# david-gimeno/tailored-avsr

Measured on AMD Instinct MI355X. Metric: utterances/sec fwd+bwd, 12L tailored AV-Branchformer (Conv3d+ResNet-18 lip frontend, fusion, CTC+6L decoder), 4 s clips, batch 32/GPU, higher is better.
Workload: dtype f32

## Files before the change

tailored-avsr_amd/csrc/gemm_conv.hip:

```cpp
#include <algorithm>
#include <vector>

#include "gemm_glds.h"

namespace tavsr {

constexpr int kOrdRuns = 80;
struct TileOrder {
  int nruns;
  int start[kOrdRuns];
  int cum[kOrdRuns + 1];
  int w[kOrdRuns];
};

__host__ __device__ inline void tile_order_map(const TileOrder& o, int b, int tiles_m, int tiles_n, int& mt, int& nt) {
  const int per = 8 * tiles_n;
  const int g = b / per, j = b - g * per, s0 = 8 * g;
  int r0 = 0;
  while (r0 + 1 < o.nruns && o.cum[r0 + 1] <= s0) ++r0;
  bool uniform = s0 + 8 <= tiles_m;
  if (uniform) {
    int r7 = r0;
    while (r7 + 1 < o.nruns && o.cum[r7 + 1] <= s0 + 7) ++r7;
    uniform = o.w[r7] == o.w[r0];
// ... 143 lines not shown
      } else {
        const int v = r / pm.n;
        pm.pos(v, y, x);
        img = r - v * pm.n;
      }
      rows.off[i] = ((int64_t)img * (d.conv_H * d.conv_W) + g.cs * y * d.conv_W + g.cs * x) * d.lda + ((q & 7) ^ ((row >> 1) & 7)) * 4;
      rows.mask[i] = pm.taps(y, x);
    }
  }
  __device__ __forceinline__ int steps() const { return nk; }
  __device__ __forceinline__ const PosMajor* row_map() const { return &pm; }
  __device__ __forceinline__ void issue(int, float* stage) {
    const tavsr_gemm_desc& d = c.d;
    const int ktap = tap, kk = tap * d.conv_C + cb * kBK;
    const int wrap = (cb + 1) * kBK >= d.conv_C;
    const uint32_t up = taps >> (tap + 1) << (tap + 1);
    cb = wrap ? 0 : cb + 1;
    tap = !wrap ? tap : up ? __builtin_ctz(up) : 9;
    rows.issue(c, c9, kk, ktap, stage);
    if constexpr (X6) LB::issue(x6_planes(d) + kk / 2, offB, stage + BM * kBK, c.wave);
    else LB::issue(c.B + (BKM ? (int64_t)kk * d.ldb : kk), offB, stage + BM * kBK, c.wave);
  }
};
template <int BM, int BN, int NT, bool BKM>
struct SourceFor<1, true, BM, BN, NT, false, BKM> {
  using type = PosMajorRowsSource<BM, BN, NT, BKM>;
};
template <int BM, int BN, int NT>
struct SourceFor<1, true, BM, BN, NT, false, false, true> {
  using type = PosMajorRowsSource<BM, BN, NT, false, true>;
};

template <int BN, int NT>
struct PatchB {
  using L = GLoader<BN, true, NT>;
  static constexpr int kDma = L::NR;
  const TileCtx& c;
  const ConvGeom g;
  int ox[L::NR], oy[L::NR], img[L::NR];
  int sb, salo, sahi, tapoff, cb, dy, dx;
  __device__ __forceinline__ explicit PatchB(const TileCtx& c_) : c(c_), g(c_.d) {
    const tavsr_gemm_desc& d = c.d;
    const int sa = kBK / g.Wo;
    sb = kBK - sa * g.Wo;
    sahi = sa / g.Ho;
    salo = sa - sahi * g.Ho;
    const int tap = c.n0 / d.conv_C;
    cb = c.n0 - tap * d.conv_C;
    dy = g.c9 ? tap / 3 - 1 : 0;
    dx = g.c9 ? tap % 3 - 1 : 0;
    tapoff = dy * d.conv_W + dx;
#pragma unroll
    for (int i = 0; i < L::NR; ++i) {
      const int m = c.kbeg + (i * NT + c.tid) / (BN / 4);
      const int t = m / g.Wo;
      ox[i] = m - t * g.Wo;
      img[i] = t / g.Ho;
      oy[i] = t - img[i] * g.Ho;
    }
  }
  __device__ __forceinline__ void issue(int, float* dst) {
    const tavsr_gemm_desc& d = c.d;
#pragma unroll
    for (int i = 0; i < L::NR; ++i) {
      const int r = (((i * NT + c.tid) % (BN / 4)) * 4);
      const int x = ox[i] * g.cs + g.p0, y = oy[i] * g.cs + g.p0;
      const bool ok = (unsigned)(y + dy) < (unsigned)d.conv_H && (unsigned)(x + dx) < (unsigned)d.conv_W;
      const int64_t pix = (int64_t)(img[i] * d.conv_H + y) * d.conv_W + x;
      dma16(ok ? c.B + (pix + tapoff) * d.conv_C + cb + r : d.conv_zero, dst + (i * NT + c.wave * 64) * 4);
      int nx = ox[i] + sb;
      const int w1 = nx >= g.Wo ? 1 : 0;
      nx -= w1 ? g.Wo : 0;
      int ny = oy[i] + salo + w1;
      const int w2 = ny >= g.Ho ? 1 : 0;
      ny -= w2 ? g.Ho : 0;
      ox[i] = nx; oy[i] = ny; img[i] += sahi + w2;
    }
  }
};
template <int BM, int BN, int NT>
struct SourceFor<2, false, BM, BN, NT, true, true> {
  using type = PairSource<PlainOperand<BM, true, NT, false>, PatchB<BN, NT>, BM>;
};

template <int BM, int BN, int NT>
struct PatchWalkSource : SourceDefaults {
  using LA = GLoader<BM, true, NT>;
  using LB = GLoader<BN, true, NT>;
  static constexpr int kDma = LA::NR + LB::NR;
  const TileCtx& c;
  const ConvGeom g;
  int64_t offA[LA::NR];
  int tapoff, cb, dy, dx;
  int n, i0, nk;
  int v = 0, img = 0, x = 0, y = 0;
  __device__ __forceinline__ static int rowsum_n0(const tavsr_gemm_desc& d) { return 4 * d.conv_C; }
  __device__ __forceinline__ bool ok(int py, int px) const {
    return (unsigned)(g.cs * py + dy) < (unsigned)c.d.conv_H && (unsigned)(g.cs * px + dx) < (unsigned)c.d.conv_W;
  }
  __device__ __forceinline__ explicit PatchWalkSource(const TileCtx& c_) : c(c_), g(c_.d) {
    const tavsr_gemm_desc& d = c.d;
    const int tap = c.n0 / d.conv_C;
    cb = c.n0 - tap * d.conv_C;
    dy = g.c9 ? tap / 3 - 1 : 0;
    dx = g.c9 ? tap % 3 - 1 : 0;
    tapoff = dy * d.conv_W + dx;
    const int P = g.Ho * g.Wo;
    i0 = c.kbeg / P;
    n = (c.kend - c.kbeg) / P;
    LA::offsets(d.lda, c.m0, d.M, c.tid, offA);
#pragma unroll
    for (int i = 0; i < LA::NR; ++i) offA[i] -= (int64_t)((i * NT + c.tid) / (BM / 4)) * d.lda;
    if (n % kBK == 0) {
      int ny = 0, nx = 0;
      for (int py = 0; py < g.Ho; ++py) ny += (unsigned)(g.cs * py + dy) < (unsigned)d.conv_H;
      for (int px = 0; px < g.Wo; ++px) nx += (unsigned)(g.cs * px + dx) < (unsigned)d.conv_W;
      nk = (n / kBK) * ny * nx;
    } else {
      nk = 0;
      int prev = 0, py = 0, px = 0;
      for (int pv = 0; pv < P; ++pv) {
        if (ok(py, px)) {
          const int s_lo = max(pv * n / kBK, prev), s_hi = ((pv + 1) * n - 1) / kBK + 1;
          if (s_hi > s_lo) { nk += s_hi - s_lo; prev = s_hi; }
        }
        if (++px == g.Wo) { px = 0; ++py; }
      }
    }
  }
  __device__ __forceinline__ int steps() const { return nk; }
  __device__ __forceinline__ void advance() {
    img += kBK;
    while (img >= n) {
      img -= n;
      ++v;
      if (++x == g.Wo) { x = 0; ++y; }
    }
  }
  __device__ __forceinline__ int64_t locate(int kl, int& py, int& px, int& pimg) const {
    int pv = v;
    pimg = img + kl;
    py = y; px = x;
    while (pimg >= n) {
      pimg -= n;
      ++pv;
      if (++px == g.Wo) { px = 0; ++py; }
    }
    pimg += i0;
    return (int64_t)pimg * (g.Ho * g.Wo) + pv;
  }
  __device__ __forceinline__ void issue(int, float* stage) {
    const tavsr_gemm_desc& d = c.d;
    for (;;) {
      bool any = false;
      int end = img + kBK, py = y, px = x;
      for (;;) {
        any |= ok(py, px);
        if (end <= n) break;
        end -= n;
        if (++px == g.Wo) { px = 0; ++py; }
      }
      if (any) break;
      advance();
    }
#pragma unroll
    for (int i = 0; i < LA::NR; ++i) {
      int py, px, pimg;
      const int64_t pix = locate((i * NT + c.tid) / (BM / 4), py, px, pimg);
      dma16(c.A + pix * d.lda + offA[i], stage + (i * NT + c.wave * 64) * 4);
    }
#pragma unroll
    for (int i = 0; i < LB::NR; ++i) {
      const int r = (((i * NT + c.tid) % (BN / 4)) * 4);
      int py, px, pimg;
      locate((i * NT + c.tid) / (BN / 4), py, px, pimg);
      const int64_t pix = ((int64_t)pimg * d.conv_H + g.cs * py) * d.conv_W + g.cs * px;
      dma16(ok(py, px) ? c.B + (pix + tapoff) * d.conv_C + cb + r : d.conv_zero, stage + BM * kBK + (i * NT + c.wave * 64) * 4);
    }
    advance();
  }
};
template <int BM, int BN, int NT>
struct SourceFor<2, true, BM, BN, NT, true, true> {
  using type = PatchWalkSource<BM, BN, NT>;
};

struct StemGeom {
  int T, H, W, Ho, Wo;
  __device__ __forceinline__ explicit StemGeom(const tavsr_gemm_desc& d)
      : T(d.conv_C), H(d.conv_H), W(d.conv_W), Ho((d.conv_H - 1) / 2 + 1), Wo((d.conv_W - 1) / 2 + 1) {}
};

template <int BM, int NT>
struct Stem4A {
  static_assert(NT == 256, "the two-taps-per-thread decoding assumes 8 rows per gather instruction");
  static constexpr int kDma = BM * kBK / NT;
  const TileCtx& c;
  const StemGeom g;
  int base[kDma], mask[kDma];
  int kk0, kk1;
  __device__ __forceinline__ explicit Stem4A(const TileCtx& c_) : c(c_), g(c_.d) {
    const int p = c.tid & 31;
    kk0 = ((((p >> 2) ^ (c.wave & 7))) << 2) + (p & 3);
    kk1 = ((((p >> 2) ^ ((c.wave + 4) & 7))) << 2) + (p & 3);
#pragma unroll
    for (int i = 0; i < kDma; ++i) {
      const int row = i * 8 + (c.tid >> 5);
      const int m = min(c.m0 + row, c.d.M - 1);
      const int wo = m % g.Wo, ho = (m / g.Wo) % g.Ho, ft = m / (g.Wo * g.Ho);
      const int t = ft % g.T, hy = 2 * ho - 3, wx = 2 * wo - 3;
      base[i] = (ft * g.H + hy) * g.W + wx;
      int mk = 0;
#pragma unroll
      for (int q = 0; q < 5; ++q) mk |= (int)((unsigned)(t + q - 2) < (unsigned)g.T) << q;
#pragma unroll
      for (int q = 0; q < 7; ++q)
        mk |= ((int)((unsigned)(hy + q) < (unsigned)g.H) << (8 + q)) | ((int)((unsigned)(wx + q) < (unsigned)g.W) << (16 + q));
      mask[i] = mk;
    }
  }
  __device__ __forceinline__ void issue(int kt, float* img) {
    int tapoff[2], sh[2];
#pragma unroll
    for (int q = 0; q < 2; ++q) {
      const int k = c.kbeg + kt * kBK + (q ? kk1 : kk0);
      const int a = k / 49, r = k - 49 * a, b = r / 7, cc = r - 7 * b;
      tapoff[q] = ((a - 2) * g.H + b) * g.W + cc;
      sh[q] = k < 245 ? (a | ((8 + b) << 8) | ((16 + cc) << 16)) : -1;
    }
#pragma unroll
    for (int i = 0; i < kDma; ++i) {
      const int q = i & 1, mk = mask[i];
      const bool ok = sh[q] >= 0 && (((mk >> (sh[q] & 31)) & (mk >> ((sh[q] >> 8) & 31)) & (mk >> ((sh[q] >> 16) & 31))) & 1);
      dma4(ok ? c.A + (base[i] + tapoff[q]) : c.d.conv_zero, img + i * NT + c.wave * 64);
    }
  }
};
template <int BM, int BN, int NT>
struct SourceFor<4, false, BM, BN, NT, false, false> {
  using type = PairSource<Stem4A<BM, NT>, PlainOperand<BN, false, NT, true>, BM>;
};

template <int BN, int NT>
struct Stem5B {
  static_assert(BN == 64 && NT == 256, "one k row per wave instruction");
  static constexpr int kDma = BN * kBK / NT;
  const TileCtx& c;
  const StemGeom g;
  int wo, ho, t, off, tapoff, c3, a, b;
  bool nok;
  bool th;
  __device__ __forceinline__ bool frame_row_ok() const {
    return nok && (unsigned)(t + a - 2) < (unsigned)g.T && (unsigned)(2 * ho - 3 + b) < (unsigned)g.H;
  }
  __device__ __forceinline__ explicit Stem5B(const TileCtx& c_) : c(c_), g(c_.d) {
    const int nn = c.n0 + (c.tid & 63);
    a = nn / 49; b = (nn % 49) / 7;
    const int cc = nn % 7;
    c3 = cc - 3;
    nok = nn < 245;
    tapoff = ((a - 2) * g.H + b - 3) * g.W + cc - 3;
    const int m = c.kbeg + c.wave;
    wo = m % g.Wo; ho = (m / g.Wo) % g.Ho;
    const int ft = m / (g.Wo * g.Ho);
    t = ft % g.T;
    off = (ft * g.H + 2 * ho) * g.W + 2 * wo;
    th = frame_row_ok();
  }
// ... 65 lines not shown
  static constexpr int kDma = L::NR;
  const TileCtx& c;
  const PaddedStemGeom g;
  int wo[L::NR], ho[L::NR], t[L::NR], off[L::NR];
  int tapoff;
  __device__ __forceinline__ explicit Stem7B(const TileCtx& c_) : c(c_), g(c_.d) {
    constexpr int CPR = BN / 4;
    int ch = (c.n0 >> 2) + (c.tid % CPR);
    if (ch >= 72) ch = 0;
    const int r = ch >> 1, a = r / 7, b = r - 7 * a;
    tapoff = (a * g.Hp + b) * g.Wp + 4 * (ch & 1);
#pragma unroll
    for (int i = 0; i < L::NR; ++i) {
      const int m = c.kbeg + (i * NT + c.tid) / CPR;
      wo[i] = m % g.Wo; ho[i] = (m / g.Wo) % g.Ho; t[i] = (m / (g.Wo * g.Ho)) % g.T;
      off[i] = g.pixel(m);
    }
  }
  __device__ __forceinline__ void issue(int, float* img) {
    constexpr int STEP = 32;
#pragma unroll
    for (int i = 0; i < L::NR; ++i) {
      dma16(c.B + (off[i] + tapoff), img + (i * NT + c.wave * 64) * 4);
      wo[i] += STEP;
      off[i] += 2 * STEP;
      while (wo[i] >= g.Wo) {
        wo[i] -= g.Wo;
        off[i] += 2 * g.Wp - 2 * g.Wo;
        if (++ho[i] == g.Ho) {
          ho[i] = 0;
          off[i] += (g.Hp - 2 * g.Ho) * g.Wp;
          if (++t[i] == g.T) { t[i] = 0; off[i] += (g.Tp - g.T) * g.Hp * g.Wp; }
        }
      }
    }
  }
};
template <int BM, int BN, int NT>
struct SourceFor<7, false, BM, BN, NT, true, true> {
  using type = PairSource<PlainOperand<BM, true, NT, false>, Stem7B<BN, NT>, BM>;
};

struct GemmArgsOrd {
  GemmArgs g;
  TileOrder ord;
};
template <int CONV, bool PM>
struct TileMap<CONV, PM, true> {
  __device__ __forceinline__ static const GemmArgs& map(const GemmArgsOrd& x, int& bid, int& zidx) {
    bid = xcd_remap(blockIdx.x, gridDim.x);
    zidx = blockIdx.z;
    if (x.ord.nruns > 0) {
      int mt, nt;
      tile_order_map(x.ord, blockIdx.x, x.g.tiles_m, x.g.tiles_n, mt, nt);
      bid = mt * x.g.tiles_n + nt;
    }
    return x.g;
  }
  __device__ __forceinline__ static const GemmArgs& map(const GemmArgs& args, int& bid, int& zidx) {
    bid = xcd_remap(blockIdx.x, gridDim.x);
    zidx = blockIdx.z;
    if (args.zmap) {
      const int tiles = gridDim.x, l = blockIdx.x + tiles * blockIdx.z, j = l >> 3;
      int zs = j / tiles;
      bid = j % tiles;
      if constexpr (PM && CONV == 2) {
        if (!(args.d.conv_posmajor & 2)) {
          if (args.n_big > 0) dw_xcd_order(j, args.tiles_m, args.tiles_n, args.nsplit >> 3, zs, bid);
          bid = dw_tile_order(bid, args.tiles_m, args.tiles_n, args.d.conv_H, args.d.conv_W);
        }
      }
      zidx = (l & 7) + 8 * zs;
    }
    return args;
  }
};

static int conv_ho(const tavsr_gemm_desc& d) { return (d.conv_H - 1) / std::max(d.conv_stride, 1) + 1; }
static int conv_wo(const tavsr_gemm_desc& d) { return (d.conv_W - 1) / std::max(d.conv_stride, 1) + 1; }

constexpr int kPmStride2MaxPos = 36;
static bool conv_pm(const tavsr_gemm_desc& d) {
  const bool stride_ok = d.conv_stride <= 1 || (d.conv_stride == 2 && (d.conv_posmajor & 8) && conv_ho(d) * conv_wo(d) <= kPmStride2MaxPos);
  return (d.conv_posmajor & ~kConvX6) && (d.conv_mode == 1 || d.conv_mode == 2) && stride_ok && (d.conv_taps == 0 || d.conv_taps == 9) &&
         (d.conv_mode == 2 || !d.a_rowsum);
}

static void tile_order_build(const tavsr_gemm_desc& d, int BM, int nsplit, TileOrder& o) {
  o.nruns = 0;
  const int cs = std::max(d.conv_stride, 1);
  const int P = conv_ho(d) * conv_wo(d);
  if (nsplit != 1 || (d.conv_posmajor & 2) || P <= 0 || d.M < P) return;
  struct Key { int H, W, cs, M, BM; };
  static thread_local Key last{0, 0, 0, 0, 0};
  static thread_local TileOrder last_o;
  if (last.H == d.conv_H && last.W == d.conv_W && last.cs == cs && last.M == d.M && last.BM == BM) { o = last_o; return; }
  PosMajor pm{};
  pm.H = conv_ho(d); pm.W = conv_wo(d); pm.n = d.M / P;
  pm.st = cs; pm.HI = d.conv_H; pm.WI = d.conv_W;
  std::vector<uint32_t> tp(P);
  for (int v = 0; v < P; ++v) {
    int y, x;
    pm.pos(v, y, x);
    tp[v] = pm.taps(y, x);
  }
  struct Run { int start, len, w; };
  std::vector<Run> runs;
  const int tiles_m = cdiv(d.M, BM);
  for (int i = 0; i < tiles_m; ++i) {
    const int vlo = (int)((int64_t)i * BM / pm.n);
    const int vhi = std::min((int)(std::min<int64_t>((int64_t)i * BM + BM - 1, d.M - 1) / pm.n), P - 1);
    uint32_t mk = 0;
    for (int v = vlo; v <= vhi; ++v) mk |= tp[v];
    const int w = __builtin_popcount(mk);
    if (!runs.empty() && runs.back().w == w) ++runs.back().len;
    else runs.push_back(Run{i, 1, w});
    if ((int)runs.size() > kOrdRuns) return;
  }
  std::stable_sort(runs.begin(), runs.end(), [](const Run& a, const Run& b) { return a.w > b.w; });
  int cum = 0;
  for (size_t r = 0; r < runs.size(); ++r) {
    o.start[r] = runs[r].start; o.cum[r] = cum; o.w[r] = runs[r].w;
    cum += runs[r].len;
  }
  o.cum[runs.size()] = cum;
  o.nruns = (int)runs.size();
  last = Key{d.conv_H, d.conv_W, cs, d.M, BM};
  last_o = o;
}

template <int BM, int BN, int MINW, bool AK, bool BKM, int CONV, bool PM, bool X6 = false, int WM = 2, int WN = 2, int S = 2>
static int launch_conv_tile(const tavsr_gemm_desc& d, const Plan& p, hipStream_t s) {
  const int zmap = (CONV == 2 || CONV == 5 || CONV == 7) && p.nsplit >= 8 && p.nsplit % 8 == 0;
  const bool two = PM && CONV == 2;
  GemmArgs a{d, p.kchunk, p.nsplit, cdiv(d.M, BM), cdiv(d.N, BN), (int)vec_epi_ok(d), zmap, two ? p.n_big : 0, two ? p.kunit : 0};
  const dim3 grid(a.tiles_m * a.tiles_n, 1, p.nsplit);
  if constexpr (PM && CONV == 1) {
    GemmArgsOrd ao{a, {}};
    tile_order_build(d, BM, p.nsplit, ao.ord);
    hipLaunchKernelGGL((gemm_glds_kernel<BM, BN, WM, WN, S, MINW, AK, BKM, 1, CONV, true, X6>), grid, dim3(WM * WN * 64), 0, s, ao);
  } else {
    hipLaunchKernelGGL((gemm_glds_kernel<BM, BN, WM, WN, S, MINW, AK, BKM, 1, CONV, PM, X6>), grid, dim3(WM * WN * 64), 0, s, a);
  }
  TAVSR_LAUNCH_CHECK();
  return launch_epilogue(a, s);
}

template <int BM, int BN, int MINW, bool AK, bool BKM, int CONV, bool X6 = false, int WM = 2, int WN = 2, int S = 2>
static int launch_conv_pm(const tavsr_gemm_desc& d, const Plan& p, hipStream_t s) {
  return conv_pm(d) ? launch_conv_tile<BM, BN, MINW, AK, BKM, CONV, true, X6, WM, WN, S>(d, p, s)
                    : launch_conv_tile<BM, BN, MINW, AK, BKM, CONV, false, X6, WM, WN, S>(d, p, s);
}

static bool conv_x6(const tavsr_gemm_desc& d, const Plan& p) {
  return (d.conv_posmajor & kConvX6) && d.conv_mode == 1 && !d.a_kmajor && !d.b_kmajor && d.ldb == d.K &&
         (d.conv_taps == 0 || d.conv_taps == 9 || (d.conv_taps == 1 && d.K >= 256)) && aligned16(d.B) && (int64_t)d.N * d.K * 6 < (1ll << 31);
}

int launch_conv(const tavsr_gemm_desc& d, const Plan& p, hipStream_t s) {
  switch (d.conv_mode) {
    case 1:
      if (d.b_kmajor) return launch_conv_pm<64, 64, 5, false, true, 1>(d, p, s);
      if (conv_x6(d, p)) {
        const bool big = p.nsplit == 1 && (int64_t)cdiv(d.M, 128) * cdiv(d.N, d.N % 128 == 0 ? 128 : 64) >= 512;
        if (big && d.N % 128 == 0) return launch_conv_pm<128, 128, 2, false, false, 1, true>(d, p, s);
        if (big) return launch_conv_pm<128, 64, 2, false, false, 1, true, 4, 1>(d, p, s);
        if (p.nsplit == 1 && d.N % 128 == 0) return launch_conv_pm<64, 128, 2, false, false, 1, true>(d, p, s);
        return launch_conv_pm<64, 64, 4, false, false, 1, true>(d, p, s);
      }
      if (p.nsplit == 1 && d.N % 128 == 0) return launch_conv_pm<64, 128, 3, false, false, 1>(d, p, s);
      return launch_conv_pm<64, 64, 5, false, false, 1>(d, p, s);
    case 2:
      if (d.M % 128 == 0) return launch_conv_pm<128, 64, 3, true, true, 2>(d, p, s);
      return launch_conv_pm<64, 64, 5, true, true, 2>(d, p, s);
    case 4: return launch_conv_tile<64, 64, 5, false, false, 4, false>(d, p, s);
    case 5: return launch_conv_tile<64, 64, 5, true, true, 5, false>(d, p, s);
    case 6: return launch_conv_tile<64, 64, 5, false, false, 6, false>(d, p, s);
    default: return launch_conv_tile<64, 64, 5, true, true, 7, false>(d, p, s);
  }
}

Plan plan_conv(const tavsr_gemm_desc& d, bool can_split, int force_split) {
  Plan pc = plan(d, can_split, true);
  if ((d.conv_mode == 2 || d.conv_mode == 5 || d.conv_mode == 7) && can_split) {
    const bool wide = d.conv_mode == 2 && d.M % 128 == 0;
    const long tiles = (long)cdiv(d.M, wide ? 128 : 64) * cdiv(d.N, 64);
    constexpr long target64 = 2560L;
    constexpr long target128 = 2304L;
    const long target = wide ? target128 : target64;
    int unit = 32;
    if (conv_pm(d)) {
      const int P = conv_ho(d) * conv_wo(d);
      int g = P, b = 32;
      while (b) { const int t = g % b; g = b; b = t; }
      unit = P / g * 32;
      if (pc.nsplit > 1) {
        pc.kchunk = cdiv(pc.kchunk, unit) * unit;
        pc.nsplit = cdiv(d.K, pc.kchunk);
      }
    }
    const long want = std::min<long>(std::max<long>(1, target / tiles), d.K / 512);
    if (want > pc.nsplit) {
      pc.kchunk = cdiv(cdiv(d.K, want), unit) * unit;
      pc.nsplit = cdiv(d.K, pc.kchunk);
    }
    if (pc.nsplit >= 16 && pc.nsplit % 8 != 0) {
      for (long w8 = pc.nsplit / 8 * 8; w8 >= 8; w8 -= 8) {
        const int kc = cdiv(cdiv(d.K, w8), unit) * unit;
        if (cdiv(d.K, kc) % 8 == 0) { pc.kchunk = kc; pc.nsplit = cdiv(d.K, kc); break; }
        if (w8 < pc.nsplit / 2) break;
      }
    }
    if (conv_pm(d) && d.conv_mode == 2 && !(d.conv_posmajor & 4) && d.K % unit == 0) {
      const long U = d.K / unit, round4 = (wide ? 768 : 1280) / 4;
      const long w = std::min<long>(force_split > 0 ? force_split : want, U) / 8 * 8;
      const bool missed = target - (long)pc.nsplit * tiles > round4, hits = target - w * tiles <= round4;
      if (w >= 8 && U % w != 0 && (force_split > 0 || (missed && hits))) {
        pc.nsplit = (int)w;
        pc.kchunk = (int)(U / w) * unit;
        pc.n_big = (int)(U % w);
        pc.kunit = unit;
      }
    }
  }
  return pc;
}

}

extern "C" int tavsr_conv_tile_order(int H, int W, int images, int bm, int tiles_n, int32_t* tile_m, int32_t* tile_n, int max_blocks) {
  using namespace tavsr;
  if (H <= 0 || W <= 0 || images <= 0 || bm <= 0 || tiles_n <= 0) return 0;
  tavsr_gemm_desc d{};
  d.conv_H = H; d.conv_W = W; d.M = images * H * W; d.conv_posmajor = 1;
  TileOrder o;
  tile_order_build(d, bm, 1, o);
  if (o.nruns == 0) return 0;
  const int tiles_m = cdiv(d.M, bm), nwg = tiles_m * tiles_n;
  for (int b = 0; b < nwg && b < max_blocks; ++b) tile_order_map(o, b, tiles_m, tiles_n, tile_m[b], tile_n[b]);
  return nwg;
}

extern "C" int tavsr_conv_dw_tile_order(int H, int W, int tiles_m, int tiles_n, int32_t* tile, int max_tiles) {
  if (H <= 0 || W <= 0 || tiles_m <= 0 || tiles_n <= 0) return 0;
  for (int q = 0; q < tiles_m * tiles_n && q < max_tiles; ++q) tile[q] = tavsr::dw_tile_order(q, tiles_m, tiles_n, H, W);
  return tiles_m * tiles_n;
}

extern "C" int tavsr_conv_dw_plan(int H, int W, int cin, int cout, int images, int posmajor, int force_split, int32_t* out) {
  using namespace tavsr;
  if (H <= 0 || W <= 0 || cin <= 0 || cout <= 0 || images <= 0 || !out) return 0;
  tavsr_gemm_desc d{};
  d.conv_mode = 2; d.conv_H = H; d.conv_W = W; d.conv_C = cin; d.conv_stride = 1; d.conv_taps = 9; d.conv_posmajor = posmajor;
  d.M = cout; d.N = 9 * cin; d.K = images * H * W; d.a_kmajor = d.b_kmajor = 1; d.nb1 = d.nb2 = 1;
  const Plan p = plan_conv(d, true, force_split);
  out[0] = p.kchunk; out[1] = p.n_big; out[2] = p.kunit;
  return p.nsplit;
}

extern "C" int tavsr_conv_dw_xcd_order(int H, int W, int tiles_m, int tiles_n, int ns, int32_t* slice, int32_t* tile, int max_tiles) {
  if (H <= 0 || W <= 0 || tiles_m <= 0 || tiles_n <= 0 || ns <= 0) return 0;
  for (int j = 0; j < ns * tiles_m * tiles_n && j < max_tiles; ++j) {
    int zs, q;
    tavsr::dw_xcd_order(j, tiles_m, tiles_n, ns, zs, q);
    slice[j] = zs;
    tile[j] = tavsr::dw_tile_order(q, tiles_m, tiles_n, H, W);
  }
  return ns * tiles_m * tiles_n;
}

#ifdef TAVSR_GEMM_TRACE
namespace tavsr {
int conv_trace_read(unsigned long long* out, int max_rows) { return trace_read_unit(out, max_rows); }
}
#endif
```

tailored-avsr_amd/csrc/gemm_glds.h:

```cpp
#pragma once
#include <type_traits>

#include "common.h"

namespace tavsr {

typedef float f32x16 __attribute__((ext_vector_type(16)));
constexpr int kBK = 32;

struct GemmArgs {
  tavsr_gemm_desc d;
  int kchunk;
  int nsplit;
  int tiles_m, tiles_n;
  int vec_epi;
  int zmap;
  int n_big, kunit;
};

template <int ROWS, int BK, bool KMAJOR>
struct Tile {
  static constexpr int LD = KMAJOR ? (ROWS + 4) : (BK + 4);
  static constexpr int SIZE = KMAJOR ? BK * LD : ROWS * LD;
};
// ... 386 lines not shown
  static constexpr int NR = ROWS * 12 / NT;
  static_assert(ROWS * 12 % NT == 0 && (ROWS * 4) % 64 == 0, "a wave instruction stays inside one plane");
  __device__ static __forceinline__ void offsets(int K, int row0, int nrows, int tid, int (&off)[NR]) {
#pragma unroll
    for (int i = 0; i < NR; ++i) {
      const int q = i * NT + tid, plane = q / (ROWS * 4), r = q % (ROWS * 4);
      const int row = r >> 2, cl = (r & 3) ^ ((row >> 2) & 3);
      off[i] = (plane * nrows + min(row0 + row, nrows - 1)) * (K / 2) + cl * 4;
    }
  }
  __device__ static __forceinline__ void issue(const float* __restrict__ gk, const int (&off)[NR], float* __restrict__ img, int wave) {
#pragma unroll
    for (int i = 0; i < NR; ++i)
      __builtin_amdgcn_global_load_lds((glb_float*)(gk + off[i]), (lds_float*)(img + (i * NT + wave * 64) * 4), 16, 0, 0);
  }
};
template <int ROWS>
__device__ __forceinline__ uint4 read_plane(const float* __restrict__ s, int p, int row, int b, int lk) {
  return *reinterpret_cast<const uint4*>(s + ((p * ROWS + row) * 4 + ((2 * b + lk) ^ ((row >> 2) & 3))) * 4);
}

template <int N>
__device__ __forceinline__ void wait_vmcnt() {
  asm volatile("s_waitcnt vmcnt(%0)" ::"n"(N) : "memory");
}

#ifdef TAVSR_GEMM_TRACE
constexpr int kTraceMax = 1 << 15;
static __device__ unsigned long long g_trace[kTraceMax][6];
static __device__ unsigned int g_trace_n;
#define TAVSR_TRACE_DECL unsigned long long tr_t[4], tr_c[4]; tr_t[0] = wall_clock64(); tr_t[1] = tr_t[0]; tr_c[1] = tr_c[2] = 0;
#define TAVSR_TRACE_AT(i) { tr_t[i] = wall_clock64(); tr_c[i] = __builtin_readcyclecounter(); }
static int trace_read_unit(unsigned long long* out, int max_rows) {
  unsigned int n = 0;
  if (hipDeviceSynchronize() != hipSuccess) return -1;
  if (hipMemcpyFromSymbol(&n, HIP_SYMBOL(g_trace_n), sizeof(n)) != hipSuccess) return -1;
  int rows = (int)(n < (unsigned)kTraceMax ? n : kTraceMax);
  if (rows > max_rows) rows = max_rows;
  if (rows > 0 && hipMemcpyFromSymbol(out, HIP_SYMBOL(g_trace), (size_t)rows * 6 * sizeof(unsigned long long)) != hipSuccess) return -1;
  n = 0;
  if (hipMemcpyToSymbol(HIP_SYMBOL(g_trace_n), &n, sizeof(n)) != hipSuccess) return -1;
  return rows;
}
int conv_trace_read(unsigned long long* out, int max_rows);
#else
#define TAVSR_TRACE_DECL
#define TAVSR_TRACE_AT(i)
#endif

struct TileCtx {
  const tavsr_gemm_desc& d;
  const float* A;
  const float* B;
  int m0, n0;
  int kbeg, kend;
  int tid, wave;
};

struct SourceDefaults {
  static constexpr bool kPosMajorRows = false;
  __device__ __forceinline__ const PosMajor* row_map() const { return nullptr; }
  __device__ __forceinline__ static int rowsum_n0(const tavsr_gemm_desc&) { return 0; }
  __device__ __forceinline__ void fix_last(float*, int, int, int) const {}
};

template <int ROWS, bool KMAJOR, int NT, bool B_SIDE>
struct PlainOperand {
  using L = GLoader<ROWS, KMAJOR, NT>;
  static constexpr int kDma = L::NR;
  const TileCtx& c;
  int64_t off[L::NR];
  const float* gk;
  int64_t kstep;
  __device__ __forceinline__ explicit PlainOperand(const TileCtx& c_) : c(c_) {
    const int64_t ld = B_SIDE ? c.d.ldb : c.d.lda;
    L::offsets(ld, B_SIDE ? c.n0 : c.m0, B_SIDE ? c.d.N : c.d.M, c.tid, off);
    kstep = KMAJOR ? (int64_t)kBK * ld : kBK;
    gk = (B_SIDE ? c.B : c.A) + (KMAJOR ? (int64_t)c.kbeg * ld : c.kbeg);
  }
  __device__ __forceinline__ void issue(int kt, float* img) { L::issue(gk + kt * kstep, off, img, c.wave); }
};

constexpr int kConvX6 = 16;
__device__ __forceinline__ const float* x6_planes(const tavsr_gemm_desc& d) { return d.B + (int64_t)d.N * d.K; }
template <int ROWS, int NT>
struct PlaneOperand {
  using L = PlaneLoader<ROWS, NT>;
  static constexpr int kDma = L::NR;
  const TileCtx& c;
  int off[L::NR];
  const float* gk;
  __device__ __forceinline__ explicit PlaneOperand(const TileCtx& c_) : c(c_) {
    L::offsets(c.d.K, c.n0, c.d.N, c.tid, off);
    gk = x6_planes(c.d) + c.kbeg / 2;
  }
  __device__ __forceinline__ void issue(int kt, float* img) { L::issue(gk + kt * (kBK / 2), off, img, c.wave); }
};

template <class HA, class HB, int BM>
struct PairSource : SourceDefaults {
  static constexpr int kDma = HA::kDma + HB::kDma;
  HA a;
  HB b;
  int nk;
  __device__ __forceinline__ explicit PairSource(const TileCtx& c) : a(c), b(c), nk((c.kend - c.kbeg) / kBK) {}
  __device__ __forceinline__ int steps() const { return nk; }
  __device__ __forceinline__ void issue(int kt, float* stage) {
    a.issue(kt, stage);
    b.issue(kt, stage + BM * kBK);
  }
};

template <int CONV, bool PM, int BM, int BN, int NT, bool AK, bool BKM, bool X6 = false>
struct SourceFor;
template <int BM, int BN, int NT, bool AK, bool BKM>
struct SourceFor<0, false, BM, BN, NT, AK, BKM> {
  using type = PairSource<PlainOperand<BM, AK, NT, false>, PlainOperand<BN, BKM, NT, true>, BM>;
};

template <int BM, int BN, int WM, int WN, int S, bool AK, bool BKM, int KW = 1, int CONV = 0, bool PM = false, bool X6 = false>
__device__ __forceinline__ void glds_tile(const tavsr_gemm_desc& d, int kchunk, int nsplit, int tiles_n, int bid, bool vec_epi,
                                          int zidx, int n_big = 0, int kunit = 0) {
  constexpr int BK = kBK, NG = BK / 8;
  static_assert(NG % KW == 0, "k-groups must divide over the wave sets");
  static_assert(!PM || KW == 1, "position-major order: one wave set");
  static_assert(!X6 || (CONV == 1 && !AK && !BKM && KW == 1), "split operands: CONV 1, both operands k-contiguous, one wave set");
  constexpr int NT = WM * WN * KW * 64;
  constexpr int TM = BM / WM / 32, TN = BN / WN / 32;
  using Src = typename SourceFor<CONV, PM, BM, BN, NT, AK, BKM, X6>::type;
  constexpr int ASZ = BM * BK, STAGE = BM * BK + BN * (X6 ? kX6RowFloats : BK);
  constexpr int G = Src::kDma;
  static_assert((S - 2) * G <= 63, "vmcnt field");
  __shared__ __attribute__((aligned(1024))) float smem[S * STAGE];

  const int tid = threadIdx.x;
  const int lane = tid & 63;
  const int wave = __builtin_amdgcn_readfirstlane(tid >> 6);
  const int kw = wave / (WM * WN), w2 = wave % (WM * WN);
  const int wm = w2 / WN, wn = w2 % WN;
  const int lr = lane & 31, lk = lane >> 5;

  TAVSR_TRACE_DECL
  const int m0 = (bid / tiles_n) * BM;
  const int n0 = (bid % tiles_n) * BN;
  const int z1 = blockIdx.y / d.nb2, z2 = blockIdx.y % d.nb2;
  const float* A = d.A + z1 * d.sA1 + z2 * d.sA2;
  const float* B = d.B + z1 * d.sB1 + z2 * d.sB2;
  const int64_t coff = z1 * d.sC1 + z2 * d.sC2;

  f32x16 acc[TM][TN];
#pragma unroll
  for (int i = 0; i < TM; ++i)
#pragma unroll
    for (int j = 0; j < TN; ++j)
#pragma unroll
      for (int r = 0; r < 16; ++r) acc[i][j][r] = 0.f;
  float asum[TM];
#pragma unroll
  for (int i = 0; i < TM; ++i) asum[i] = 0.f;
  float bpre[TN];
#pragma unroll
  for (int j = 0; j < TN; ++j) {
    const int n = n0 + wn * TN * 32 + j * 32 + lr;
    bpre[j] = (d.bias && nsplit == 1 && n < d.N) ? d.bias[n] : 0.f;
  }

  const int kbeg = zidx * kchunk + min(zidx, n_big) * kunit;
  const int kend = min(d.K, kbeg + kchunk + (zidx < n_big ? kunit : 0));
  const TileCtx ctx{d, A, B, m0, n0, kbeg, kend, tid, wave};
  Src src(ctx);
  const int nk = src.steps();
  const bool want_rowsum = d.a_rowsum != nullptr && n0 == Src::rowsum_n0(d) && wn == 0;

  const int arow = wm * TM * 32 + lr, brow = wn * TN * 32 + lr;
  auto compute = [&](int st) {
    const float* a_s = smem + st * STAGE;
    const float* b_s = a_s + ASZ;
    if constexpr (X6) {
      float af[2][TM][8];
      uint4 bq[2][TN][3];
      auto read_block = [&](int b, float (&fa)[TM][8], uint4 (&qb)[TN][3]) {
#pragma unroll
        for (int i = 0; i < TM; ++i) {
          float lo[4], hi[4];
          read_frag_g<BM, false>(a_s, arow + i * 32, 2 * b, lk, lo);
          read_frag_g<BM, false>(a_s, arow + i * 32, 2 * b + 1, lk, hi);
#pragma unroll
          for (int e = 0; e < 4; ++e) { fa[i][e] = lo[e]; fa[i][4 + e] = hi[e]; }
        }
#pragma unroll
        for (int j = 0; j < TN; ++j)
#pragma unroll
          for (int p = 0; p < 3; ++p) qb[j][p] = read_plane<BN>(b_s, p, brow + j * 32, b, lk);
      };
      read_block(0, af[0], bq[0]);
#pragma unroll
      for (int b = 0; b < BK / 16; ++b) {
        const int c = b & 1;
        if (b + 1 < BK / 16) read_block(b + 1, af[c ^ 1], bq[c ^ 1]);
        GEMM_SB();
        uint4 ah[TM], am[TM], al[TM];
#pragma unroll
        for (int i = 0; i < TM; ++i) split_frag(af[c][i], ah[i], am[i], al[i]);
#pragma unroll
        for (int pr = 0; pr < 6; ++pr) {
          constexpr int PA[6] = {0, 2, 1, 0, 1, 0}, PB[6] = {2, 0, 1, 1, 0, 0};
#pragma unroll
          for (int i = 0; i < TM; ++i)
#pragma unroll
            for (int j = 0; j < TN; ++j)
              acc[i][j] = mfma_bf16(PA[pr] == 0 ? ah[i] : PA[pr] == 1 ? am[i] : al[i], bq[c][j][PB[pr]], acc[i][j]);
        }
#pragma unroll
        for (int i = 0; i < TM; ++i)
          asum[i] += ((af[c][i][0] + af[c][i][1]) + (af[c][i][2] + af[c][i][3])) + ((af[c][i][4] + af[c][i][5]) + (af[c][i][6] + af[c][i][7]));
        GEMM_SB();
      }
      return;
    }
    float af[2][TM][4], bf[2][TN][4];
#pragma unroll
    for (int i = 0; i < TM; ++i) read_frag_g<BM, AK>(a_s, arow + i * 32, kw, lk, af[0][i]);
#pragma unroll
    for (int j = 0; j < TN; ++j) read_frag_g<BN, BKM>(b_s, brow + j * 32, kw, lk, bf[0][j]);
#pragma unroll
    for (int q = 0; q < NG / KW; ++q) {
      const int c = q & 1;
      if (q + 1 < NG / KW) {
#pragma unroll
        for (int i = 0; i < TM; ++i) read_frag_g<BM, AK>(a_s, arow + i * 32, kw + (q + 1) * KW, lk, af[c ^ 1][i]);
#pragma unroll
        for (int j = 0; j < TN; ++j) read_frag_g<BN, BKM>(b_s, brow + j * 32, kw + (q + 1) * KW, lk, bf[c ^ 1][j]);
      }
      GEMM_SB();
#pragma unroll
      for (int kk = 0; kk < 4; ++kk)
#pragma unroll
        for (int i = 0; i < TM; ++i)
#pragma unroll
          for (int j = 0; j < TN; ++j)
            acc[i][j] = __builtin_amdgcn_mfma_f32_32x32x2f32(af[c][i][kk], bf[c][j][kk], acc[i][j], 0, 0, 0);
#pragma unroll
      for (int i = 0; i < TM; ++i) asum[i] += (af[c][i][0] + af[c][i][1]) + (af[c][i][2] + af[c][i][3]);
      GEMM_SB();
    }
  };

#pragma unroll
  for (int j = 0; j < S - 1; ++j)
    if (j < nk) src.issue(j, smem + j * STAGE);
  int st = 0;
  int kt = 0;
  for (; kt + S - 1 < nk; ++kt) {
    wait_vmcnt<(S - 2) * G>();
    __builtin_amdgcn_s_barrier();
#ifdef TAVSR_GEMM_TRACE
    if (kt == 0) TAVSR_TRACE_AT(1)
#endif
    const int sn = st == 0 ? S - 1 : st - 1;
    src.issue(kt + S - 1, smem + sn * STAGE);
    compute(st);
// ... 121 lines not shown
```

tailored-avsr_amd/tavsr/ops/__init__.py:

```python
from __future__ import annotations

import os
from typing import Optional

PROFILE: Optional[GemmProfile] = None

WGRAD_BESIDE = os.environ.get("TAVSR_WGRAD_BESIDE", "1") != "0"
WGRAD_SLOT = int(os.environ.get("TAVSR_WGRAD_SLOT", "0"))

LN_BWD_DROP = True

ATTN_FUSED = True

FASTATTN_LIMIT = "1 <= attention_heads <= 8, size <= 512, size / attention_heads a multiple of 4"

FFN2 = True
FFN2_BWD = True
FFN2_BWD_LN = os.environ.get("TAVSR_FFN2_BWD_LN", "1") != "0"

LAYER_C = os.environ.get("TAVSR_LAYER_C", "1") != "0"
LAYER_C_EAGER_ONLY = os.environ.get("TAVSR_LAYER_C", "1") != "capture"
BLOCKS_C = os.environ.get("TAVSR_BLOCKS_C", "1") != "0"

CSGU_FUSED = True
CSGU_STATS_IN_GEMM = True
CGMLP_ACT_BWD_FUSED = True

MERGE_ROWS = True
MERGE_PROJ = os.environ.get("TAVSR_MERGE_PROJ", "1") == "1"
MERGE_ROWDOT = True

STEM_IMPLICIT = True
STEM_PAD16 = True

CONV_TAPSKIP = os.environ.get("TAVSR_CONV_TAPSKIP", "1") != "0"
CONV_TAPSKIP_MAXPOS = int(os.environ.get("TAVSR_CONV_TAPSKIP_MAXPOS", "121"))
CONV_TILEORDER = os.environ.get("TAVSR_CONV_TILEORDER", "1") != "0"
CONV_TAPSKIP_MAXPOS_DW = int(os.environ.get("TAVSR_CONV_TAPSKIP_MAXPOS_DW", "36"))
CONV_DW_UNEVEN = os.environ.get("TAVSR_CONV_DW_UNEVEN", "1") != "0"

CONV_TAPSKIP_STRIDE2 = os.environ.get("TAVSR_CONV_TAPSKIP_STRIDE2", "1") != "0"
CONV_TAPSKIP_STRIDE2_DW = os.environ.get("TAVSR_CONV_TAPSKIP_STRIDE2_DW", "0") != "0"
CONV_TAPSKIP_STRIDE2_MAXPOS = 36
CONV_X6 = os.environ.get("TAVSR_CONV_X6", "1") != "0"

CTC_ALIGN_CHUNK = 16

RESAMPLE_ROLLOFF, RESAMPLE_ZEROS, RESAMPLE_BETA = 0.9475937167399596, 64, 14.769656459379492

ROWLIN = True
ROWLIN_KSPLIT = 4
TREE_ROWS_MAX_KEYS = 1024
RNNT_SEARCH_KINDS = {"alsd": 0, "tsd": 1}
RNNT_SEARCH_LIMIT = ("1 <= beam <= 64, beam < vocabulary, at least one frame, u_max >= 0, 1 <= max_sym_exp <= 8, the trie of an "
                     "utterance within 2^30 words")

RNNT_WS_FLOATS = 1 << 24

from .base import *
from .rng import *
from .streams import *
from .data import *
from .blocks import *
from .matmul import *
from .norm import *
from .attention import *
from .fastattn import *
from .vision import *
from .losses import *
from .search import *
from .rnnt import *
```

tailored-avsr_amd/tavsr/ops/vision.py:

```python
from __future__ import annotations

import torch

from .. import ops
from .._lib import ACT, check, lib, ptr, require_cuda, stream
from .base import empty
from .matmul import gemm

__all__ = ["conv1_fwd", "conv1_bwd", "im2col3x3s2", "col2im3x3s2_relu", "conv_out", "im2col2d", "col2im2d", "stem_implicit_ok",
           "stem_pad16_ok", "stem_pad", "stem_weight_288", "stem_weight_grad_from_288", "stem_conv_fwd_pad16", "stem_conv_dw_pad16",
           "stem_conv_fwd", "stem_conv_dw", "im2col_stem", "bn_stats", "rsqrt_eps", "bn_apply_fwd", "bn_bwd", "bn_bwd_pooled",
           "maxpool3x3s2_fwd", "bn_act_maxpool3x3s2_fwd", "maxpool3x3s2_bwd", "avgpool_fwd", "avgpool_bwd", "conv_wflip", "conv_wsplit", "x6_takes", "_tapskip",
           "_tapskip2", "_tapskip_any", "conv3x3_fwd", "conv3x3_dx", "conv3x3_dw"]


def conv1_fwd(x, w, bias):
    B, T, F = x.shape
    Cn = w.shape[0]
    To, Fo = (T - 3) // 2 + 1, (F - 3) // 2 + 1
    y = empty(B, To, Fo, Cn, like=x)
    require_cuda(x, w, bias)
    check(lib().tavsr_conv1_fwd(ptr(x), ptr(w), ptr(bias), ptr(y), B, T, F, Cn, stream()), "tavsr_conv1_fwd")
    return y


def conv1_bwd(dz, x, Cn):
    B, T, F = x.shape
    dw, db = empty(Cn, 9, like=x), empty(Cn, like=x)
    ws = empty(lib().tavsr_conv1_bwd_ws(B, T, F, Cn), like=x)
    check(lib().tavsr_conv1_bwd(ptr(dz), ptr(x), ptr(dw), ptr(db), 0, ptr(ws), B, T, F, Cn, stream()), "tavsr_conv1_bwd")
    return dw, db


def im2col3x3s2(y):
    B, Ti, Fi, Cn = y.shape
    To, Fo = (Ti - 3) // 2 + 1, (Fi - 3) // 2 + 1
    col = empty(B * To * Fo, 9 * Cn, like=y)
    check(lib().tavsr_im2col3x3s2(ptr(y), ptr(col), B, Ti, Fi, Cn, stream()), "tavsr_im2col3x3s2")
    return col, To, Fo


def col2im3x3s2_relu(dcol, yrelu):
    B, Ti, Fi, Cn = yrelu.shape
    dz = torch.empty_like(yrelu)
    check(lib().tavsr_col2im3x3s2_relu(ptr(dcol), ptr(yrelu), ptr(dz), B, Ti, Fi, Cn, stream()), "tavsr_col2im3x3s2_relu")
    return dz


def conv_out(n, k, s, p):
    return (n + 2 * p - k) // s + 1


def im2col2d(x, N, H, W, Cn, KH, KW, stride, pad):
    require_cuda(x)
    Ho, Wo = conv_out(H, KH, stride, pad), conv_out(W, KW, stride, pad)
    col = empty(N * Ho * Wo, KH * KW * Cn, like=x)
    check(lib().tavsr_im2col2d(ptr(x), ptr(col), N, H, W, Cn, KH, KW, stride, pad, stream()), "tavsr_im2col2d")
    return col, Ho, Wo


def col2im2d(dcol, N, H, W, Cn, KH, KW, stride, pad, extra=None):
    require_cuda(dcol, extra)
    assert extra is None or (extra.is_contiguous() and extra.shape == (dcol.shape[0], Cn))
    dx = empty(N * H * W, Cn, like=dcol)
    check(lib().tavsr_col2im2d(ptr(dcol), ptr(dx), N, H, W, Cn, KH, KW, stride, pad, ptr(extra), stream()), "tavsr_col2im2d")
    return dx


def stem_implicit_ok(x) -> bool:
    B, T, H, W = x.shape
    Ho, Wo = conv_out(H, 7, 2, 3), conv_out(W, 7, 2, 3)
    return (ops.STEM_IMPLICIT and H % 2 == 0 and W % 2 == 0 and W >= 8 and (B * T * Ho * Wo) % 32 == 0 and T < 1024 and H < 1000 and W < 1000
            and B * T * H * W < 2 ** 31 and x.data_ptr() % 16 == 0)


def stem_pad16_ok(x) -> bool:
    B, T, H, W = x.shape
    Ho, Wo = H // 2, W // 2
    return (ops.STEM_IMPLICIT and ops.STEM_PAD16 and H % 2 == 0 and W % 4 == 0 and (B * T * Ho * Wo) % 32 == 0
            and B * (T + 5) * (H + 6) * (W + 8) < 2 ** 31)


def stem_pad(x):
    return torch.nn.functional.pad(x, (3, 5, 3, 3, 2, 3)).contiguous()


def stem_weight_288(w):
    co = w.shape[0]
    return torch.nn.functional.pad(torch.nn.functional.pad(w.reshape(co, 35, 7), (0, 1)).reshape(co, 280), (0, 8)).contiguous()


def stem_weight_grad_from_288(g, shape):
    co = g.shape[0]
    return g[:, :280].reshape(co, 35, 8)[:, :, :7].reshape(shape).contiguous()

# ... 68 lines not shown
    M, Cn = x.shape
    require_cuda(dy, x, mean, rstd, gamma, beta, res)
    assert need_dz or res is None
    dz, dx = (torch.empty_like(x) if need_dz else None), torch.empty_like(x)
    dg, db = empty(Cn, like=x), empty(Cn, like=x)
    ws = empty(lib().tavsr_bn_ws(M, Cn), like=x)
    check(lib().tavsr_bn_bwd(ptr(dy), ptr(x), ptr(mean), ptr(rstd), ptr(gamma), ptr(beta), ptr(res), ptr(dz), ptr(dx), ptr(dg), ptr(db), M,
                             Cn, ACT[act], ptr(ws), stream()), "tavsr_bn_bwd")
    return dz, dx, dg, db


def bn_bwd_pooled(dpool, idx, x, mean, rstd, gamma, beta, N, H, W, act=None):
    M, Cn = x.shape
    require_cuda(dpool, idx, x, mean, rstd, gamma, beta)
    assert M == N * H * W and dpool.is_contiguous() and idx.dtype == torch.uint8 and idx.is_contiguous()
    dx = torch.empty_like(x)
    dg, db = empty(Cn, like=x), empty(Cn, like=x)
    ws = empty(lib().tavsr_bn_ws(M, Cn), like=x)
    check(lib().tavsr_bn_bwd_pooled(ptr(dpool), ptr(idx), ptr(x), ptr(mean), ptr(rstd), ptr(gamma), ptr(beta), ptr(dx), ptr(dg), ptr(db), N,
                                    H, W, Cn, ACT[act], ptr(ws), stream()), "tavsr_bn_bwd_pooled")
    return dx, dg, db


def maxpool3x3s2_fwd(x, N, H, W, Cn):
    Ho, Wo = conv_out(H, 3, 2, 1), conv_out(W, 3, 2, 1)
    y = empty(N * Ho * Wo, Cn, like=x)
    idx = torch.empty((N * Ho * Wo, Cn), dtype=torch.uint8, device=x.device)
    check(lib().tavsr_maxpool3x3s2_fwd(ptr(x), ptr(y), ptr(idx), N, H, W, Cn, stream()), "tavsr_maxpool3x3s2_fwd")
    return y, idx, Ho, Wo


def bn_act_maxpool3x3s2_fwd(z, mean, rstd, gamma, beta, act, N, H, W, Cn):
    Ho, Wo = conv_out(H, 3, 2, 1), conv_out(W, 3, 2, 1)
    require_cuda(z, mean, rstd, gamma, beta)
    y = empty(N * Ho * Wo, Cn, like=z)
    idx = torch.empty((N * Ho * Wo, Cn), dtype=torch.uint8, device=z.device)
    check(lib().tavsr_bn_act_maxpool3x3s2_fwd(ptr(z), ptr(mean), ptr(rstd), ptr(gamma), ptr(beta), ACT[act], ptr(y), ptr(idx), N, H, W, Cn,
                                              stream()), "tavsr_bn_act_maxpool3x3s2_fwd")
    return y, idx, Ho, Wo


def maxpool3x3s2_bwd(dy, idx, N, H, W, Cn):
    dx = empty(N * H * W, Cn, like=dy)
    check(lib().tavsr_maxpool3x3s2_bwd(ptr(dy), ptr(idx), ptr(dx), N, H, W, Cn, stream()), "tavsr_maxpool3x3s2_bwd")
    return dx


def avgpool_fwd(x, N, P, Cn):
    y = empty(N, Cn, like=x)
    check(lib().tavsr_avgpool_fwd(ptr(x), ptr(y), N, P, Cn, stream()), "tavsr_avgpool_fwd")
    return y


def avgpool_bwd(dy, N, P, Cn):
    dx = empty(N * P, Cn, like=dy)
    check(lib().tavsr_avgpool_bwd(ptr(dy), ptr(dx), N, P, Cn, stream()), "tavsr_avgpool_bwd")
    return dx


def conv_wflip(w2d, cout, cin):
    require_cuda(w2d)
    out = empty(cin, 9 * cout, like=w2d)
    check(lib().tavsr_conv_wflip(ptr(w2d), ptr(out), cout, cin, stream()), "tavsr_conv_wflip")
    return out


def conv_wsplit(w):
    require_cuda(w)
    N, K = w.shape
    assert w.stride(1) == 1 and K % 16 == 0
    out = empty(5 * N * K // 2, like=w)
    check(lib().tavsr_conv_wsplit(ptr(w), w.stride(0), ptr(out), N, K, stream()), "tavsr_conv_wsplit")
    return out


def x6_takes(w, taps=9, pad0=False):
    return bool(ops.CONV_X6 and not pad0 and w.stride(1) == 1 and w.shape[1] % 32 == 0 and (taps == 9 or w.shape[1] >= 256))


def _x6(w, planes, taps=9, pad0=False):
    if not x6_takes(w, taps, pad0):
        return w, 0
    return (conv_wsplit(w) if planes is None else planes), 16


def _tapskip_bits():
    return 1 | (0 if ops.CONV_TILEORDER else 2) | (0 if ops.CONV_DW_UNEVEN else 4)


def _tapskip(H, W, stride=1, taps=9, pad0=False, dw=False):
    on = ops.CONV_TAPSKIP and stride == 1 and taps == 9 and not pad0 and H * W <= (ops.CONV_TAPSKIP_MAXPOS_DW if dw else ops.CONV_TAPSKIP_MAXPOS)
    return _tapskip_bits() if on else 0


def _tapskip2(H, W, dw=False):
    on = ops.CONV_TAPSKIP and (ops.CONV_TAPSKIP_STRIDE2_DW if dw else ops.CONV_TAPSKIP_STRIDE2)
    return (_tapskip_bits() | 8) if on and ((H - 1) // 2 + 1) * ((W - 1) // 2 + 1) <= ops.CONV_TAPSKIP_STRIDE2_MAXPOS else 0


def _tapskip_any(H, W, stride, taps, pad0, dw=False):
    return _tapskip2(H, W, dw) if stride == 2 and taps == 9 and not pad0 else _tapskip(H, W, stride, taps, pad0, dw)


def conv3x3_fwd(x, w2d, H, W, stride=1, taps=9, pad0=False, bias=None, act=None, planes=None):
    M, cin = x.shape
    cout = w2d.shape[0]
    if pad0:
        assert taps == 9
        Ho, Wo = (H - 3) // stride + 1, (W - 3) // stride + 1
    else:
        Ho, Wo = (H - 1) // stride + 1, (W - 1) // stride + 1
    Mo = M // (H * W) * Ho * Wo
    z = empty(Mo, cout, like=x)
    B, x6 = _x6(w2d, planes, taps, pad0)
    gemm(Mo, cout, taps * cin, x, cin, B, taps * cin, z, cout, conv=(1, H, W, cin, stride, 90 if pad0 else taps, _tapskip_any(H, W, stride, taps, pad0) | x6),
         bias=bias, act=act)
    return z


def conv3x3_dx(dz, wflip, H, W, res=None, planes=None):
    M, cout = dz.shape
    cin = wflip.shape[0]
    dx = empty(M, cin, like=dz)
    B, x6 = _x6(wflip, planes)
    gemm(M, cin, 9 * cout, dz, cout, B, 9 * cout, dx, cin, conv=(1, H, W, cout, 0, 0, _tapskip(H, W) | x6), R=res, ldr=0 if res is None else cin)
    return dx


def conv3x3_dw(dz, x, H, W, stride=1, taps=9, pad0=False, bias_grad=False, force=None):
    M, cout = dz.shape
    cin = x.shape[1]
    dw = empty(cout, taps * cin, like=dz)
    gb = empty(cout, like=dz) if bias_grad else None
    gemm(cout, taps * cin, M, dz, cout, x, cin, dw, taps * cin, a_kmajor=True, b_kmajor=True,
         conv=(2, H, W, cin, stride, 90 if pad0 else taps, _tapskip_any(H, W, stride, taps, pad0, dw=True)), a_rowsum=gb, force=force)
    return (dw, gb) if bias_grad else dw
```

Baseline: 453.5.

## Use split-bf16 x6 MFMA path for conv weight-gradient GEMMs

```diff
diff --git a/tailored-avsr_amd/csrc/gemm_conv.hip b/tailored-avsr_amd/csrc/gemm_conv.hip
--- a/tailored-avsr_amd/csrc/gemm_conv.hip
+++ b/tailored-avsr_amd/csrc/gemm_conv.hip
@@ -249,6 +249,10 @@
 struct SourceFor<2, false, BM, BN, NT, true, true> {
   using type = PairSource<PlainOperand<BM, true, NT, false>, PatchB<BN, NT>, BM>;
 };
+template <int BM, int BN, int NT>
+struct SourceFor<2, false, BM, BN, NT, true, true, true> {
+  using type = PairSource<PlainOperand<BM, true, NT, false>, PatchB<BN, NT>, BM>;
+};
 
 template <int BM, int BN, int NT>
 struct PatchWalkSource : SourceDefaults {
@@ -351,6 +355,10 @@
 struct SourceFor<2, true, BM, BN, NT, true, true> {
   using type = PatchWalkSource<BM, BN, NT>;
 };
+template <int BM, int BN, int NT>
+struct SourceFor<2, true, BM, BN, NT, true, true, true> {
+  using type = PatchWalkSource<BM, BN, NT>;
+};
 
 struct StemGeom {
   int T, H, W, Ho, Wo;
@@ -582,7 +590,7 @@
 constexpr int kPmStride2MaxPos = 36;
 static bool conv_pm(const tavsr_gemm_desc& d) {
   const bool stride_ok = d.conv_stride <= 1 || (d.conv_stride == 2 && (d.conv_posmajor & 8) && conv_ho(d) * conv_wo(d) <= kPmStride2MaxPos);
-  return (d.conv_posmajor & ~kConvX6) && (d.conv_mode == 1 || d.conv_mode == 2) && stride_ok && (d.conv_taps == 0 || d.conv_taps == 9) &&
+  return (d.conv_posmajor & ~(kConvX6 | kConvX6Dw)) && (d.conv_mode == 1 || d.conv_mode == 2) && stride_ok && (d.conv_taps == 0 || d.conv_taps == 9) &&
          (d.conv_mode == 2 || !d.a_rowsum);
 }
 
@@ -657,6 +665,16 @@
          (d.conv_taps == 0 || d.conv_taps == 9 || (d.conv_taps == 1 && d.K >= 256)) && aligned16(d.B) && (int64_t)d.N * d.K * 6 < (1ll << 31);
 }
 
+static bool conv_x6_dw(const tavsr_gemm_desc& d, const Plan&) {
+  return (d.conv_posmajor & kConvX6Dw) && d.conv_mode == 2 && d.a_kmajor && d.b_kmajor && (d.conv_taps == 0 || d.conv_taps == 9 || d.conv_taps == 1);
+}
+
+struct DwTile { int bm, bn, waves, x6; };
+static DwTile conv_dw_tile(const tavsr_gemm_desc& d, const Plan& p) {
+  const int x6 = conv_x6_dw(d, p);
+  return d.M % 128 == 0 ? DwTile{128, 64, 4, x6} : DwTile{64, 64, 4, x6};
+}
+
 int launch_conv(const tavsr_gemm_desc& d, const Plan& p, hipStream_t s) {
   switch (d.conv_mode) {
     case 1:
@@ -670,9 +688,13 @@
       }
       if (p.nsplit == 1 && d.N % 128 == 0) return launch_conv_pm<64, 128, 3, false, false, 1>(d, p, s);
       return launch_conv_pm<64, 64, 5, false, false, 1>(d, p, s);
-    case 2:
-      if (d.M % 128 == 0) return launch_conv_pm<128, 64, 3, true, true, 2>(d, p, s);
+    case 2: {
+      const DwTile t = conv_dw_tile(d, p);
+      if (t.x6 && t.bm == 128) return launch_conv_pm<128, 64, 3, true, true, 2, true>(d, p, s);
+      if (t.x6) return launch_conv_pm<64, 64, 5, true, true, 2, true>(d, p, s);
+      if (t.bm == 128) return launch_conv_pm<128, 64, 3, true, true, 2>(d, p, s);
       return launch_conv_pm<64, 64, 5, true, true, 2>(d, p, s);
+    }
     case 4: return launch_conv_tile<64, 64, 5, false, false, 4, false>(d, p, s);
     case 5: return launch_conv_tile<64, 64, 5, true, true, 5, false>(d, p, s);
     case 6: return launch_conv_tile<64, 64, 5, false, false, 6, false>(d, p, s);
@@ -758,6 +780,19 @@
   return p.nsplit;
 }
 
+extern "C" int tavsr_conv_dw_tile(int H, int W, int cin, int cout, int images, int stride, int taps, int posmajor, int32_t* out) {
+  using namespace tavsr;
+  if (H <= 0 || W <= 0 || cin <= 0 || cout <= 0 || images <= 0 || stride <= 0 || !out) return 0;
+  tavsr_gemm_desc d{};
+  d.conv_mode = 2; d.conv_H = H; d.conv_W = W; d.conv_C = cin; d.conv_stride = stride; d.conv_taps = taps; d.conv_posmajor = posmajor;
+  const int p0 = taps == 90 ? 1 : 0, nt = taps == 1 ? 1 : 9;
+  d.M = cout; d.N = nt * cin; d.K = images * ((H - 1 - 2 * p0) / stride + 1) * ((W - 1 - 2 * p0) / stride + 1);
+  d.a_kmajor = d.b_kmajor = 1; d.nb1 = d.nb2 = 1;
+  const DwTile t = conv_dw_tile(d, plan_conv(d, true, 0));
+  out[0] = t.bm; out[1] = t.bn; out[2] = t.waves; out[3] = t.x6;
+  return 1;
+}
+
 extern "C" int tavsr_conv_dw_xcd_order(int H, int W, int tiles_m, int tiles_n, int ns, int32_t* slice, int32_t* tile, int max_tiles) {
   if (H <= 0 || W <= 0 || tiles_m <= 0 || tiles_n <= 0 || ns <= 0) return 0;
   for (int j = 0; j < ns * tiles_m * tiles_n && j < max_tiles; ++j) {
diff --git a/tailored-avsr_amd/csrc/gemm_glds.h b/tailored-avsr_amd/csrc/gemm_glds.h
--- a/tailored-avsr_amd/csrc/gemm_glds.h
+++ b/tailored-avsr_amd/csrc/gemm_glds.h
@@ -492,6 +492,7 @@
 };
 
 constexpr int kConvX6 = 16;
+constexpr int kConvX6Dw = 32;
 __device__ __forceinline__ const float* x6_planes(const tavsr_gemm_desc& d) { return d.B + (int64_t)d.N * d.K; }
 template <int ROWS, int NT>
 struct PlaneOperand {
@@ -534,11 +535,12 @@
   constexpr int BK = kBK, NG = BK / 8;
   static_assert(NG % KW == 0, "k-groups must divide over the wave sets");
   static_assert(!PM || KW == 1, "position-major order: one wave set");
-  static_assert(!X6 || (CONV == 1 && !AK && !BKM && KW == 1), "split operands: CONV 1, both operands k-contiguous, one wave set");
+  static_assert(!X6 || (KW == 1 && ((CONV == 1 && !AK && !BKM) || (CONV == 2 && AK && BKM))),
+                "split operands: CONV 1 with both operands k-contiguous or CONV 2 with both k-major, one wave set");
   constexpr int NT = WM * WN * KW * 64;
   constexpr int TM = BM / WM / 32, TN = BN / WN / 32;
   using Src = typename SourceFor<CONV, PM, BM, BN, NT, AK, BKM, X6>::type;
-  constexpr int ASZ = BM * BK, STAGE = BM * BK + BN * (X6 ? kX6RowFloats : BK);
+  constexpr int ASZ = BM * BK, STAGE = BM * BK + BN * (X6 && !AK ? kX6RowFloats : BK);
   constexpr int G = Src::kDma;
   static_assert((S - 2) * G <= 63, "vmcnt field");
   __shared__ __attribute__((aligned(1024))) float smem[S * STAGE];
@@ -586,7 +588,54 @@
   auto compute = [&](int st) {
     const float* a_s = smem + st * STAGE;
     const float* b_s = a_s + ASZ;
-    if constexpr (X6) {
+    if constexpr (X6 && AK) {
+      float af[2][TM][8], bf[2][TN][8];
+      auto read_block = [&](int b, float (&fa)[TM][8], float (&fb)[TN][8]) {
+#pragma unroll
+        for (int i = 0; i < TM; ++i) {
+          float lo[4], hi[4];
+          read_frag_g<BM, true>(a_s, arow + i * 32, 2 * b, lk, lo);
+          read_frag_g<BM, true>(a_s, arow + i * 32, 2 * b + 1, lk, hi);
+#pragma unroll
+          for (int e = 0; e < 4; ++e) { fa[i][e] = lo[e]; fa[i][4 + e] = hi[e]; }
+        }
+#pragma unroll
+        for (int j = 0; j < TN; ++j) {
+          float lo[4], hi[4];
+          read_frag_g<BN, true>(b_s, brow + j * 32, 2 * b, lk, lo);
+          read_frag_g<BN, true>(b_s, brow + j * 32, 2 * b + 1, lk, hi);
+#pragma unroll
+          for (int e = 0; e < 4; ++e) { fb[j][e] = lo[e]; fb[j][4 + e] = hi[e]; }
+        }
+      };
+      read_block(0, af[0], bf[0]);
+#pragma unroll
+      for (int b = 0; b < BK / 16; ++b) {
+        const int c = b & 1;
+        if (b + 1 < BK / 16) read_block(b + 1, af[c ^ 1], bf[c ^ 1]);
+        GEMM_SB();
+        uint4 aq[TM][3], bq[TN][3];
+#pragma unroll
+        for (int i = 0; i < TM; ++i) split_frag(af[c][i], aq[i][0], aq[i][1], aq[i][2]);
+#pragma unroll
+        for (int j = 0; j < TN; ++j) split_frag(bf[c][j], bq[j][0], bq[j][1], bq[j][2]);
+#pragma unroll
+        for (int pr = 0; pr < 6; ++pr) {
+          constexpr int PA[6] = {0, 2, 1, 0, 1, 0}, PB[6] = {2, 0, 1, 1, 0, 0};
+#pragma unroll
+          for (int i = 0; i < TM; ++i)
+#pragma unroll
+            for (int j = 0; j < TN; ++j) acc[i][j] = mfma_bf16(aq[i][PA[pr]], bq[j][PB[pr]], acc[i][j]);
+        }
+#pragma unroll
+        for (int i = 0; i < TM; ++i) {
+          asum[i] += (af[c][i][0] + af[c][i][1]) + (af[c][i][2] + af[c][i][3]);
+          asum[i] += (af[c][i][4] + af[c][i][5]) + (af[c][i][6] + af[c][i][7]);
+        }
+        GEMM_SB();
+      }
+      return;
+    } else if constexpr (X6) {
       float af[2][TM][8];
       uint4 bq[2][TN][3];
       auto read_block = [&](int b, float (&fa)[TM][8], uint4 (&qb)[TN][3]) {
diff --git a/tailored-avsr_amd/tavsr/ops/__init__.py b/tailored-avsr_amd/tavsr/ops/__init__.py
--- a/tailored-avsr_amd/tavsr/ops/__init__.py
+++ b/tailored-avsr_amd/tavsr/ops/__init__.py
@@ -43,6 +43,7 @@
 CONV_TAPSKIP_STRIDE2_DW = os.environ.get("TAVSR_CONV_TAPSKIP_STRIDE2_DW", "0") != "0"
 CONV_TAPSKIP_STRIDE2_MAXPOS = 36
 CONV_X6 = os.environ.get("TAVSR_CONV_X6", "1") != "0"
+CONV_X6_DW = os.environ.get("TAVSR_CONV_X6_DW", "1") != "0"
 
 CTC_ALIGN_CHUNK = 16
 
diff --git a/tailored-avsr_amd/tavsr/ops/vision.py b/tailored-avsr_amd/tavsr/ops/vision.py
--- a/tailored-avsr_amd/tavsr/ops/vision.py
+++ b/tailored-avsr_amd/tavsr/ops/vision.py
@@ -10,7 +10,7 @@
 __all__ = ["conv1_fwd", "conv1_bwd", "im2col3x3s2", "col2im3x3s2_relu", "conv_out", "im2col2d", "col2im2d", "stem_implicit_ok",
            "stem_pad16_ok", "stem_pad", "stem_weight_288", "stem_weight_grad_from_288", "stem_conv_fwd_pad16", "stem_conv_dw_pad16",
            "stem_conv_fwd", "stem_conv_dw", "im2col_stem", "bn_stats", "rsqrt_eps", "bn_apply_fwd", "bn_bwd", "bn_bwd_pooled",
-           "maxpool3x3s2_fwd", "bn_act_maxpool3x3s2_fwd", "maxpool3x3s2_bwd", "avgpool_fwd", "avgpool_bwd", "conv_wflip", "conv_wsplit", "x6_takes", "_tapskip",
+           "maxpool3x3s2_fwd", "bn_act_maxpool3x3s2_fwd", "maxpool3x3s2_bwd", "avgpool_fwd", "avgpool_bwd", "conv_wflip", "conv_wsplit", "x6_takes", "x6_dw_takes", "_tapskip",
            "_tapskip2", "_tapskip_any", "conv3x3_fwd", "conv3x3_dx", "conv3x3_dw"]
 
 
@@ -245,6 +245,10 @@
     if not x6_takes(w, taps, pad0):
         return w, 0
     return (conv_wsplit(w) if planes is None else planes), 16
+
+
+def x6_dw_takes(cin, cout, taps=9, pad0=False, mode=2, pixels=0):
+    return bool(ops.CONV_X6_DW and mode == 2 and not pad0 and taps in (9, 1) and pixels % 32 == 0 and cin % 64 == 0)
 
 
 def _tapskip_bits():
@@ -295,6 +299,7 @@
     cin = x.shape[1]
     dw = empty(cout, taps * cin, like=dz)
     gb = empty(cout, like=dz) if bias_grad else None
+    x6 = 32 if x6_dw_takes(cin, cout, taps, pad0, pixels=M) else 0
     gemm(cout, taps * cin, M, dz, cout, x, cin, dw, taps * cin, a_kmajor=True, b_kmajor=True,
-         conv=(2, H, W, cin, stride, 90 if pad0 else taps, _tapskip_any(H, W, stride, taps, pad0, dw=True)), a_rowsum=gb, force=force)
+         conv=(2, H, W, cin, stride, 90 if pad0 else taps, _tapskip_any(H, W, stride, taps, pad0, dw=True) | x6), a_rowsum=gb, force=force)
     return (dw, gb) if bias_grad else dw
```

Result: faster. 468.4, median of 6 (+3.3%).
